# grantjr1842/delayed-streams-modeling

Measured on AMD Instinct MI355X. Metric: real-time stream throughput, stt-1b-en_fr @ bs=64 per GPU (Mimi encode + LM decode per 80 ms frame), higher is better.
Workload: dtype bf16 weights + bf16 KV, f32 activations as three exact bf16 pieces, f32 accumulate (v_mfma_f32_16x16x32_bf16); 1 GPU; stt-1b-en_fr batch=64 streaming, ring KV cache full (750 frames), Mimi encode + LM decode HIP path; streams_per_gpu=64, parallelism=replicas x1 (independent stream batches, no per-step collective), streams=encoder stream || 2 LM group stream(s)

## Files before the change

delayed-streams-modeling_amd/csrc/dsm_device.h:

```cpp
#pragma once
#include <hip/hip_runtime.h>

#include <atomic>
#include <cstdarg>
#include <cstdio>
#include <cstdlib>
#include <deque>
#include <mutex>
#include <shared_mutex>
#include <string>
#include <vector>

#include "../../include/dsm.h"
#include "dsm_gemm_plan.h"

#define HIPCHK_E(eng, expr)                                                                         \
  do {                                                                                              \
    hipError_t _e = (expr);                                                                         \
    if (_e != hipSuccess) {                                                                         \
      (eng)->set_error("%s failed: %s (%s:%d)", #expr, hipGetErrorString(_e), __FILE__, __LINE__);  \
      return DSM_ERR_DEVICE;                                                                        \
    }                                                                                               \
  } while (0)
#define HIPCHK(expr) HIPCHK_E(e, expr)

static void dsm_read_env(struct DsmDevice* e, bool stt);

struct DsmDevice {
  int device = 0;
  bool opened = false;
  hipStream_t s_enc = nullptr, s_model = nullptr;
  static constexpr int kMaxGroups = 4;
  hipStream_t s_grp[kMaxGroups] = {nullptr, nullptr, nullptr, nullptr};
  hipEvent_t ev_fork = nullptr, ev_grp_done[kMaxGroups] = {};
  bool prio_streams = false;
  int prio_hi = 0;
  bool use_graphs = true;
  bool fuse_qkv = true;
  bool stream_prio = false;
  bool fuse_front = true;
  int chunk_loop_min_tiles = GemmKnobs().chunk_loop_min_tiles;
  int loop_depth = GemmKnobs().loop_depth;
  int smallk_min_tiles = GemmKnobs().smallk_min_tiles;
  int smallk_mt = GemmKnobs().smallk_mt;
  size_t attn_lds_pad = 60000;
  int dot_mode = 0;

  int open(int device_id, int dot_mode_, bool stt) {
    device = device_id;
    dot_mode = dot_mode_;
    int ndev = 0;
    if (hipGetDeviceCount(&ndev) != hipSuccess || ndev <= device_id) {
      set_error("no usable HIP device %d (found %d): libdsm_mi355x has no CPU fallback", device_id, ndev);
      return DSM_ERR_DEVICE;
    }
    HIPCHK_E(this, hipSetDevice(device_id));
    opened = true;
    dsm_read_env(this, stt);
    prio_streams = stt;
    int prio_lo = 0;
    if (stt && stream_prio) (void)hipDeviceGetStreamPriorityRange(&prio_lo, &prio_hi);
    if (int rc = new_stream(&s_enc, prio_lo)) return rc;
    return new_stream(&s_model, prio_hi);
  }
  int new_stream(hipStream_t* out, int prio) {
    HIPCHK_E(this, prio_streams ? hipStreamCreateWithPriority(out, hipStreamNonBlocking, prio)
                                : hipStreamCreateWithFlags(out, hipStreamNonBlocking));
    return 0;
  }
  int open_groups(int G) {
    for (int g = 1; g < G; ++g) {
      if (int rc = new_stream(&s_grp[g], prio_hi)) return rc;
      if (int rc = new_event(&ev_grp_done[g])) return rc;
    }
    return new_event(&ev_fork);
  }
  int sid(hipStream_t st) const {
    if (st == s_enc) return 0;
    for (int g = 1; g < kMaxGroups; ++g)
      if (st == s_grp[g]) return 1 + g;
    return 1;
  }

  std::mutex own_mu;
  std::vector<void*> allocs, pinned;
  std::vector<hipEvent_t> events;
  template <typename T>
  int dalloc(T** out, size_t count, bool zero = true) {
    void* p = nullptr;
    size_t bytes = count * sizeof(T) + 256;
    HIPCHK_E(this, hipMalloc(&p, bytes));
    {
      std::lock_guard<std::mutex> lk(own_mu);
      allocs.push_back(p);
    }
    if (zero) {
      HIPCHK_E(this, hipMemset(p, 0, bytes));
      HIPCHK_E(this, hipStreamSynchronize(nullptr));
    }
    *out = reinterpret_cast<T*>(p);
    return 0;
  }
  template <typename T>
  int upload(T** out, const T* host, size_t count) {
    if (int rc = dalloc(out, count)) return rc;
    HIPCHK_E(this, hipMemcpy(*out, host, count * sizeof(T), hipMemcpyHostToDevice));
    HIPCHK_E(this, hipStreamSynchronize(nullptr));
    return 0;
  }
  template <typename T>
  int halloc(T** out, size_t count) {
    void* p = nullptr;
    HIPCHK_E(this, hipHostMalloc(&p, count * sizeof(T)));
    std::lock_guard<std::mutex> lk(own_mu);
    pinned.push_back(p);
    *out = reinterpret_cast<T*>(p);
    return 0;
  }
  int new_event(hipEvent_t* out, unsigned flags = hipEventDisableTiming) {
    HIPCHK_E(this, hipEventCreateWithFlags(out, flags));
    std::lock_guard<std::mutex> lk(own_mu);
    events.push_back(*out);
    return 0;
// ... 178 lines not shown
```

delayed-streams-modeling_amd/csrc/dsm_engine.hip:

```cpp
#include <hip/hip_runtime.h>

#include <cmath>
#include <cstdarg>
#include <cstdio>
#include <cstdlib>
#include <cstring>
#include <atomic>
#include <mutex>
#include <shared_mutex>
#include <string>
#include <set>
#include <vector>

#include "../../include/dsm.h"
#include "dsm_device.h"
#include "dsm_config_presets.h"
#include "dsm_gemm_plan.h"
#include "dsm_kernels.h"
#include "dsm_numerics.h"
#include "dsm_safetensors.h"

static thread_local std::string g_create_error;

static int dsm_env_int(const char* name, int dflt) {
  const char* v = getenv(name);
  return v ? atoi(v) : dflt;
}
static void dsm_read_env(DsmDevice* e, bool stt) {
  e->chunk_loop_min_tiles = gemm_default_knobs(stt, e->dot_mode).chunk_loop_min_tiles;
  if (stt && e->dot_mode == 1) e->attn_lds_pad = 40000;
  e->use_graphs = dsm_env_int("DSM_GRAPHS", 1) != 0;
  e->fuse_qkv = dsm_env_int("DSM_FUSE_QKV", 1) != 0;
  e->stream_prio = dsm_env_int("DSM_STREAM_PRIO", 0) != 0;
  e->fuse_front = dsm_env_int("DSM_FUSE_FRONT", 1) != 0;
  e->chunk_loop_min_tiles = dsm_env_int("DSM_CHUNK_LOOP_MIN", e->chunk_loop_min_tiles);
  e->loop_depth = dsm_env_int("DSM_LOOP_DEPTH", e->loop_depth) == 2 ? 2 : 4;
  e->smallk_min_tiles = dsm_env_int("DSM_SMALLK_MIN", e->smallk_min_tiles);
  const int mt = dsm_env_int("DSM_SMALLK_MT", e->smallk_mt);
  if (mt == 1 || mt == 2 || mt == 4) e->smallk_mt = mt;
}


namespace {

struct Linear {
  void* w = nullptr;
  float* bias = nullptr;
  int N = 0, K = 0, Npad = 0, Kpad = 0;
  bool bf16 = false;
  bool packed = false;
};

struct ConvGeom {
  Linear lin;
  int in_c = 0, out_c = 0, k = 0, stride = 1;
  int S = 0;
  int T_in = 0;
  int T_out = 0;
  bool replicate = false;
};

ConvGeom over_frames(const ConvGeom& g, int r) {
  ConvGeom c = g;
  c.T_in *= r;
  c.T_out *= r;
  return c;
}

struct TLayerW {
  Linear in_proj, out_proj, ff_in, ff_out;
  float *n1w = nullptr, *n1b = nullptr, *n2w = nullptr, *n2b = nullptr, *ls1 = nullptr, *ls2 = nullptr;
  Linear ca_q, ca_kv, ca_out;
  float *ncw = nullptr, *ncb = nullptr;
};

struct TransformerW {
  dsm_transformer_config cfg{};
  int hidden = 0;
  std::vector<TLayerW> layers;
  float* inv_freq = nullptr;
  bool rope_pos_before = false;
  bool has_ca = false;
  int ca_norm_rms = 0;
};

struct CaState {
  std::vector<void*> k, v;
  uint32_t* last = nullptr;
  uint8_t* act = nullptr;
  float* att = nullptr;
  int smax = 0;
};

struct TransformerState {
  std::vector<void*> k, v;
  uint32_t *pos = nullptr, *idx = nullptr, *start_pos = nullptr, *widx = nullptr;
  float* rope_cs = nullptr;
};

struct RvqW {
  Linear input_proj, output_proj;
  int n_q = 0;
  std::vector<Linear> codebooks;
};

struct MimiW {
  dsm_mimi_config cfg{};
  ConvGeom init_conv, final_conv, downsample;
  struct Stage {
    ConvGeom ra, rb, down;
  };
  std::vector<Stage> stages;
  TransformerW tr;
  RvqW rvq_first, rvq_rest;
  struct DecStage {
    Linear up;
    float* up_bias = nullptr;
    int in_c = 0, out_c = 0, k = 0, stride = 0, T_in = 0;
    ConvGeom ra, rb;
  };
  bool has_decoder = false;
  ConvGeom dec_init, dec_final;
  std::vector<DecStage> dec_stages;
  TransformerW dec_tr;
  float* upsample_w = nullptr;
  const float** emb_ptrs = nullptr;
};

struct ActScratch {
  float *x = nullptr, *xn = nullptr, *q = nullptr, *att = nullptr, *g = nullptr;
  ActScratch from_row(size_t r0, int d, int hid) const { return {x + r0 * d, xn + r0 * d, q + r0 * d, att + r0 * d, g + r0 * hid}; }
};

struct SeanetEnc {
  float* cat_init = nullptr;
  struct Stage {
    float *y = nullptr, *cat_ra = nullptr, *cat_rb = nullptr, *cat_down = nullptr;
  };
  std::vector<Stage> stages;
  float* cat_final = nullptr;
};

struct MimiState {
  float* pcm = nullptr;
  SeanetEnc enc;
  ActScratch act;
  float* cat_ds = nullptr;
  float* latent = nullptr;
  float *res_first = nullptr, *res_rest = nullptr, *pval = nullptr;
  uint32_t* pidx = nullptr;
  uint32_t* codes = nullptr;
  TransformerState tr;
  ConvStateDesc* descs = nullptr;
  std::vector<ConvStateDesc> h_descs;
  int ds_desc = -1;
  bool first_call = true;
  uint8_t* mask = nullptr;
};

struct MimiDecState {
  bool ready = false, first_call = true;
  DsmDevice::GraphSlot* graph = nullptr;
  float* h_pcm_out = nullptr;
  uint32_t* codes = nullptr;
  uint8_t* mask = nullptr;
  uint8_t* started = nullptr;
  float *q_first = nullptr, *q_rest = nullptr, *emb = nullptr, *up_carry = nullptr;
  ActScratch act;
  TransformerState tr;
  float* cat_init = nullptr;
  struct Stage {
    float *x = nullptr, *z = nullptr, *carry = nullptr, *y = nullptr, *cat_ra = nullptr, *cat_rb = nullptr;
  };
  std::vector<Stage> stages;
  float* cat_final = nullptr;
  float* pcm = nullptr;
  ConvStateDesc* descs = nullptr;
  std::vector<ConvStateDesc> h_descs;
};

struct LmW {
  uint16_t* text_emb = nullptr;
  uint16_t* audio_emb = nullptr;
  TransformerW tr;
  float* out_norm = nullptr;
  Linear text_linear, extra_heads;
};

struct LmState {
  ActScratch act;
  float *hidden = nullptr, *logits = nullptr, *eh = nullptr, *prs = nullptr;
  uint32_t *next_cb = nullptr, *text_token = nullptr, *text_out = nullptr, *codes_in = nullptr;
  uint8_t *first_step = nullptr, *mask = nullptr;
  uint32_t* rng_key = nullptr;
  unsigned long long* rng_pos = nullptr;
  uint8_t* gmask = nullptr;
  TransformerState tr;
  struct Group {
    int b0 = 0, nb = 0;
    TransformerState view;
  };
  std::vector<Group> groups;
};

struct HostItem {
  size_t step_idx = 0;
  std::vector<uint32_t> word_tokens;
  bool unended_word = false;
  double last_stop_time = 0.0;
};

}

struct dsm_engine : DsmDevice {
  dsm_asr_config cfg{};
  int B = 0;
  hipEvent_t ev_grp_in[kMaxGroups] = {}, ev_stagger[kMaxGroups] = {};
  bool grp_busy = false;
  bool serialize_groups = false;
  hipEvent_t ev_codes_consumed = nullptr;
  bool codes_consumed_valid = false;
  hipEvent_t ev_join = nullptr, ev_a = nullptr, ev_b = nullptr, ev_c = nullptr, ev_d = nullptr;
  MimiW mimi_w;
  MimiState mimi[2];
  std::atomic<bool> mimi1_ready{false};
  std::mutex mimi1_mu;
  MimiDecState dec;
  LmW lm_w;
  LmState lm;
  GraphSlot *g_enc[2] = {}, *g_grp[kMaxGroups] = {};
  float* h_pcm = nullptr;
// ... 787 lines not shown
```

delayed-streams-modeling_amd/csrc/dsm_engine_api.inc:

```

namespace {

template <typename KVT, int HD, int T>
int launch_attn_t(DsmDevice* e, hipStream_t st, float* out, const float* q, const void* k, const void* v,
                  const uint32_t* start_pos, const uint8_t* active, int B, int H, int ctx, int d, const AttnFused& fq) {
  constexpr int UNR = (sizeof(KVT) == 2 && T == 1 && HD == 128) ? 8 : 4;
  size_t lds = sizeof(float) * ((size_t)T * ctx + 4 * T * HD + 16);
  if ((long)B * H >= 2048 && (size_t)2 * ctx * HD * sizeof(KVT) >= (size_t)256 * 1024) lds += e->attn_lds_pad;
  if (lds > 64 * 1024) {
    static size_t allowed = 0;
    if (lds > allowed) {
      HIPCHK(hipFuncSetAttribute(reinterpret_cast<const void*>(&attn_kernel<KVT, HD, T, UNR>), hipFuncAttributeMaxDynamicSharedMemorySize, (int)lds));
      allowed = lds;
    }
  }
  const int tag = e->tag_attn[e->sid(st)];
  if (T == 1 && HD == 64 && ctx <= 32) {
    const int ph = e->prof_begin(tag, st);
    hipLaunchKernelGGL((attn_small_kernel<KVT, 64>), dim3((B * H + 3) / 4), dim3(256), 0, st, out, q, reinterpret_cast<const KVT*>(k),
                       reinterpret_cast<const KVT*>(v), start_pos, active, B * H, H, ctx, d, fq);
    e->prof_end(ph, st);
    HIPCHK(hipGetLastError());
    return 0;
  }
// ... 71 lines not shown
    a.act = 1;
    a.Y = act.g; a.ymap = plain_map(M, w.hidden);
    if (int rc = gemm_store<WT>(e, st, a)) return rc;
  }
  GemmArgs a = base_args(L.ff_out, act.g, plain_map(M, w.hidden), M);
  a.scale = L.ls2;
  a.res = act.x; a.rmap = plain_map(M, d);
  if (last && final_out) {
    a.Y = final_out; a.ymap = final_map;
  } else {
    a.Y = act.x; a.ymap = plain_map(M, d);
  }
  if (!last) set_norm(a, w.layers[l + 1].n1w, w.layers[l + 1].n1b, act.xn, c.norm);
  else if (post_norm_out) set_norm(a, post_norm_w, nullptr, post_norm_out, c.norm);
  return gemm_store<WT>(e, st, a);
}

template <typename WT, typename KVT>
int transformer_forward(DsmDevice* e, hipStream_t st, const TransformerW& w, TransformerState& s, const ActScratch& act, int B,
                        int T, const uint8_t* d_mask, float* final_out, RowMap final_map, const float* post_norm_w = nullptr,
                        float* post_norm_out = nullptr, int phase = 0, const CaState* ca = nullptr, bool head_done = false) {
  const dsm_transformer_config& c = w.cfg;
  const int d = c.d_model, H = c.num_heads, hd = d / H, M = B * T;
  if (phase != 2 && !head_done) {
    hipLaunchKernelGGL(kv_builder_kernel, dim3(B), dim3(64), 0, st, s.pos, s.idx, d_mask, s.start_pos, s.widx,
                       c.positional_embedding == 1 ? s.rope_cs : (float*)nullptr, w.inv_freq, B, T, c.context, hd,
                       w.rope_pos_before ? 1 : 0);
    HIPCHK(hipGetLastError());
    if (int rc = run_norm(e, st, act.xn, act.x, w.layers[0].n1w, w.layers[0].n1b, M, d, c.norm)) return rc;
  }
  for (int l = 0; l < c.num_layers; ++l) {
    const TLayerW& L = w.layers[l];
    AttnFused fq{};
    fq.nt = sizeof(KVT) == 2;
    if (!(phase == 2 && l == 0)) {
      GemmArgs a = base_args(L.in_proj, act.xn, plain_map(M, d), M);
      a.Y = act.q;
      a.d = d; a.hd = hd; a.H = H; a.T = T; a.ctx = c.context;
      a.kcache = s.k[l]; a.vcache = s.v[l];
      a.widx = s.widx;
      a.rope_cs = c.positional_embedding == 1 ? s.rope_cs : nullptr;
      a.active = d_mask;
      Slabs sl;
      if (int rc = launch_gemm<WT, KVT, EPI_QKV, 1>(e, st, a, true, T == 1 && e->fuse_qkv ? &sl : nullptr)) return rc;
      if (sl.ws) {
        fq.ws = sl.ws; fq.ld = sl.ld; fq.cstride = sl.cstride; fq.chunks = sl.chunks;
        fq.rope_cs = a.rope_cs;
        fq.widx = s.widx;
      }
      if (int rc = launch_attn<KVT>(e, st, act.att, act.q, s.k[l], s.v[l], s.start_pos, d_mask, B, H, hd, T, c.context, d, fq)) return rc;
    }
    if (phase == 1) return 0;
    if (int rc = transformer_layer_tail<WT, KVT>(e, st, w, l, act, B, T, final_out, final_map, post_norm_w, post_norm_out, ca)) return rc;
  }
  return 0;
}

template <typename F>
int with_kv_type(bool kv_bf16, F&& f) {
  return kv_bf16 ? f(uint16_t{}) : f(float{});
}

int fork_groups(DsmDevice* e, hipStream_t st, size_t G) {
  if (G > 1) {
    HIPCHK(hipEventRecord(e->ev_fork, st));
    for (size_t g = 1; g < G; ++g) HIPCHK(hipStreamWaitEvent(e->s_grp[g], e->ev_fork, 0));
  }
  return 0;
}
template <typename F>
int run_groups(DsmDevice* e, hipStream_t st, size_t G, bool serialize, F&& body) {
  for (size_t g = G; g-- > 0;) {
    hipStream_t gs = (g == 0 || serialize) ? st : e->s_grp[g];
    if (int rc = body(g, gs)) return rc;
    if (g > 0) HIPCHK(hipEventRecord(e->ev_grp_done[g], gs));
  }
  return 0;
}
int join_groups(DsmDevice* e, hipStream_t st, size_t G) {
  for (size_t g = 1; g < G; ++g) HIPCHK(hipStreamWaitEvent(st, e->ev_grp_done[g], 0));
  return 0;
}

int seanet_encode(DsmDevice* e, hipStream_t st, const MimiW& w, SeanetEnc& s, const float* cat_init, int B, int r, float* out,
                  RowMap omap, bool front_done = false) {
  const RowMap none = plain_map(1, 1);
  const size_t n = w.stages.size();
  const ConvGeom g0 = over_frames(w.init_conv, r), gf = over_frames(w.final_conv, r);
  if (!front_done)
    if (int rc = run_conv(e, st, g0, cat_init, B, s.stages[0].y, plain_map(B * g0.T_out, g0.out_c), s.stages[0].cat_ra,
                          cat_map(over_frames(w.stages[0].ra, r)), nullptr, none))
      return rc;
  for (size_t i = 0; i < n; ++i) {
    const ConvGeom ra = over_frames(w.stages[i].ra, r), rb = over_frames(w.stages[i].rb, r), dn = over_frames(w.stages[i].down, r);
    SeanetEnc::Stage& ss = s.stages[i];
    if (!(i == 0 && front_done)) {
      if (int rc = run_conv(e, st, ra, ss.cat_ra, B, nullptr, none, ss.cat_rb, cat_map(rb), nullptr, none)) return rc;
      if (int rc = run_conv(e, st, rb, ss.cat_rb, B, nullptr, none, ss.cat_down, cat_map(dn), ss.y, plain_map(B * rb.T_out, rb.out_c)))
        return rc;
    }
    if (i + 1 < n) {
      if (int rc = run_conv(e, st, dn, ss.cat_down, B, s.stages[i + 1].y, plain_map(B * dn.T_out, dn.out_c), s.stages[i + 1].cat_ra,
                            cat_map(over_frames(w.stages[i + 1].ra, r)), nullptr, none))
        return rc;
    } else if (int rc = run_conv(e, st, dn, ss.cat_down, B, nullptr, none, s.cat_final, cat_map(gf), nullptr, none)) {
      return rc;
    }
  }
  return run_conv(e, st, gf, s.cat_final, B, out, omap, nullptr, none, nullptr, none);
}

int mimi_encode_body(dsm_engine* e, int side, hipStream_t st);
int mimi_encode(dsm_engine* e, int side, hipStream_t st) {
  return run_captured(e, *e->g_enc[side], st, (uint64_t)e->sid(st), [&] { return mimi_encode_body(e, side, st); });
}
int mimi_encode_body(dsm_engine* e, int side, hipStream_t st) {
  const MimiW& w = e->mimi_w;
  MimiState& s = e->mimi[side];
  const int B = e->B;
  const RowMap none = plain_map(1, 1);
  e->tag_gemm[e->sid(st)] = DSM_PROF_GEMM_MIMI;
  e->tag_attn[e->sid(st)] = DSM_PROF_ATTN_MIMI;
  bool fused_front = false;
  {
    const MimiW::Stage& s0 = w.stages[0];
    const ConvGeom& c = w.init_conv;
    fused_front = e->fuse_front && c.in_c == 1 && c.k == 7 && c.stride == 1 && c.out_c == 64 && c.S == 6 && !c.lin.bf16 &&
                  s0.ra.k == 3 && s0.ra.stride == 1 && s0.ra.in_c == 64 && s0.ra.out_c == 32 && s0.ra.S == 2 && !s0.ra.lin.bf16 &&
                  s0.rb.k == 1 && s0.rb.stride == 1 && s0.rb.in_c == 32 && s0.rb.out_c == 64 && !s0.rb.lin.bf16 &&
                  c.T_in % 64 == 0 && c.T_out == c.T_in && s0.ra.T_in == c.T_in && s0.rb.T_in == c.T_in && s0.down.in_c == 64 &&
                  s0.down.T_in == c.T_in && !c.replicate && !s0.ra.replicate;
    if (fused_front) {
      SeanetFrontArgs fa;
      fa.cat_init = s.enc.cat_init;
      fa.w0 = reinterpret_cast<const float*>(c.lin.w); fa.b0 = c.lin.bias; fa.ld0 = c.lin.Kpad;
      fa.w1 = reinterpret_cast<const float*>(s0.ra.lin.w); fa.b1 = s0.ra.lin.bias; fa.ld1 = s0.ra.lin.Kpad;
      fa.w2 = reinterpret_cast<const float*>(s0.rb.lin.w); fa.b2 = s0.rb.lin.bias; fa.ld2 = s0.rb.lin.Kpad;
      fa.cat_ra = s.enc.stages[0].cat_ra;
      fa.cat_down = s.enc.stages[0].cat_down;
      fa.T = c.T_in; fa.S0 = c.S; fa.Sd = s0.down.S;
      const int ph = e->prof_begin(e->tag_gemm[e->sid(st)], st);
      hipLaunchKernelGGL(seanet_front_kernel<64>, dim3(c.T_in / 64, B), dim3(256), seanet_front_lds<64>(), st, fa);
      e->prof_end(ph, st);
      HIPCHK(hipGetLastError());
    }
  }
  const int Tt = w.final_conv.T_out, d = w.cfg.dimension;
  if (int rc = seanet_encode(e, st, w, s.enc, s.enc.cat_init, B, 1, s.act.x, plain_map(B * Tt, d), fused_front)) return rc;
  if (int rc = transformer_forward<float, float>(e, st, w.tr, s.tr, s.act, B, Tt, s.mask, s.cat_ds, cat_map(w.downsample))) return rc;
  if (s.first_call && w.downsample.S > 0) {
    hipLaunchKernelGGL(conv_replicate_init_kernel, dim3(B), dim3(256), 0, st, s.h_descs[s.ds_desc]);
    HIPCHK(hipGetLastError());
  }
  if (int rc = run_conv(e, st, w.downsample, s.cat_ds, B, s.latent, plain_map(B, d), nullptr, none, nullptr, none)) return rc;
  const int n_q = w.cfg.quantizer_n_q, qd = w.cfg.quantizer_dim;
  e->tag_gemm[e->sid(st)] = DSM_PROF_RVQ;
  for (int which = 0; which < 2; ++which) {
    const RvqW& r = which == 0 ? w.rvq_first : w.rvq_rest;
    if (r.n_q == 0) continue;
    float* res = which == 0 ? s.res_first : s.res_rest;
    {
      GemmArgs a = base_args(r.input_proj, s.latent, plain_map(B, d), B);
      a.Y = res; a.ymap = plain_map(B, qd);
      if (int rc = gemm_store<float>(e, st, a)) return rc;
    }
    for (int i = 0; i < r.n_q; ++i) {
      const Linear& cb = r.codebooks[i];
      GemmArgs a = base_args(cb, res, plain_map(B, qd), B);
      a.pval = s.pval; a.pidx = s.pidx;
      if (int rc = launch_gemm<float, float, EPI_RVQ, 1>(e, st, a, true)) return rc;
      hipLaunchKernelGGL(rvq_select_kernel, dim3(B), dim3(256), 0, st, s.pval, s.pidx, (cb.N + 15) / 16, B, s.codes, n_q,
                         which == 0 ? 0 : 1 + i, res, reinterpret_cast<const float*>(cb.w), qd, cb.Kpad);
      HIPCHK(hipGetLastError());
    }
  }
  if (!s.h_descs.empty()) {
    hipLaunchKernelGGL(conv_state_shift_kernel, dim3(B, (unsigned)s.h_descs.size()), dim3(256), 0, st, s.descs, s.mask,
                       s.first_call ? 1 : 0, nullptr);
    HIPCHK(hipGetLastError());
  }
  s.first_call = false;
  return 0;
}

int alloc_dec_state(DsmDevice* e, const MimiW& w, MimiDecState& s, int B) {
  if (s.ready) return 0;
  const dsm_mimi_config& c = w.cfg;
  const int dim = c.dimension, T2 = w.dec_init.T_in;
  if (!w.has_decoder) {
    e->set_error("the Mimi checkpoint has no decoder.* tensors: decode_step is unavailable");
    return DSM_ERR_STATE;
  }
  if (int rc = e->dalloc(&s.codes, (size_t)B * c.quantizer_n_q)) return rc;
  if (int rc = e->dalloc(&s.mask, B)) return rc;
  if (int rc = e->dalloc(&s.q_first, (size_t)B * c.quantizer_dim)) return rc;
  if (int rc = e->dalloc(&s.q_rest, (size_t)B * c.quantizer_dim)) return rc;
  if (int rc = e->dalloc(&s.emb, (size_t)B * dim)) return rc;
  if (int rc = e->dalloc(&s.up_carry, (size_t)B * c.downsample_stride * dim)) return rc;
  if (int rc = alloc_act(e, &s.act, (size_t)B * T2, dim, c.transformer.dim_feedforward)) return rc;
  if (int rc = alloc_transformer_state(e, &s.tr, c.transformer, B, T2, false)) return rc;
  auto add = [&](float* cat, const ConvGeom& g) { add_desc(s.h_descs, cat, g); };
  if (int rc = alloc_cat(e, &s.cat_init, w.dec_init, B)) return rc;
  add(s.cat_init, w.dec_init);
  s.stages.resize(w.dec_stages.size());
  for (size_t i = 0; i < w.dec_stages.size(); ++i) {
    const MimiW::DecStage& st = w.dec_stages[i];
    MimiDecState::Stage& ss = s.stages[i];
    const int T_out = st.T_in * st.stride;
    if (int rc = e->dalloc(&ss.x, (size_t)B * st.T_in * st.in_c)) return rc;
    if (int rc = e->dalloc(&ss.z, (size_t)B * st.T_in * st.k * st.out_c)) return rc;
    if (int rc = e->dalloc(&ss.carry, (size_t)B * (st.k - st.stride) * st.out_c)) return rc;
    if (int rc = e->dalloc(&ss.y, (size_t)B * T_out * st.out_c)) return rc;
    if (int rc = alloc_cat(e, &ss.cat_ra, st.ra, B)) return rc;
    if (int rc = alloc_cat(e, &ss.cat_rb, st.rb, B)) return rc;
    add(ss.cat_ra, st.ra);
    add(ss.cat_rb, st.rb);
  }
  if (int rc = alloc_cat(e, &s.cat_final, w.dec_final, B)) return rc;
  add(s.cat_final, w.dec_final);
  if (int rc = e->dalloc(&s.pcm, (size_t)B * DSM_FRAME_SIZE * c.channels)) return rc;
  if (int rc = e->upload(&s.descs, s.h_descs.data(), s.h_descs.size())) return rc;
  if (int rc = e->halloc(&s.h_pcm_out, (size_t)B * DSM_FRAME_SIZE)) return rc;
  s.graph = e->graph_slot();
  s.ready = true;
  return 0;
}

int mimi_decode_body(DsmDevice* e, const MimiW& w, MimiDecState& s, int B, hipStream_t st);
int mimi_decode(DsmDevice* e, const MimiW& w, MimiDecState& s, int B, hipStream_t st) {
  return run_captured(e, *s.graph, st, (uint64_t)e->sid(st), [&] { return mimi_decode_body(e, w, s, B, st); });
}
// ... 1017 lines not shown
  return 0;
}

int dsm_prof_timeline(dsm_engine* e, int on) {
  if (!e) return DSM_ERR_INVALID;
  e->timeline = on != 0;
  return 0;
}

int dsm_prof_timeline_read(dsm_engine* e, int* sid, int* kind, int* tag, double* start_us, double* end_us, int cap) {
  if (!e) return DSM_ERR_INVALID;
  HIPCHK(hipSetDevice(e->device));
  ApiShared api(e);
  if (int rc = dsm_sync(e)) return rc;
  const size_t n = e->dev_ts_tags.size();
  int out = 0;
  if (n) {
    std::vector<unsigned long long> h(2 * n);
    HIPCHK(hipMemcpy(h.data(), e->dev_ts, sizeof(unsigned long long) * 2 * n, hipMemcpyDeviceToHost));
    int khz = 100000;
    (void)hipDeviceGetAttribute(&khz, hipDeviceAttributeWallClockRate, e->device);
    unsigned long long t0 = ~0ull;
    for (size_t i = 0; i < n; ++i)
      if (h[2 * i + 1] >= h[2 * i] && h[2 * i] < t0) t0 = h[2 * i];
    for (size_t i = 0; i < n && out < cap; ++i) {
      if (h[2 * i + 1] < h[2 * i]) continue;
      sid[out] = e->dev_ts_info[i] >> 8;
      kind[out] = e->dev_ts_info[i] & 0xff;
      tag[out] = e->dev_ts_tags[i];
      start_us[out] = (double)(h[2 * i] - t0) * 1000.0 / khz;
      end_us[out] = (double)(h[2 * i + 1] - t0) * 1000.0 / khz;
      ++out;
    }
    for (size_t i = 0; i < n; ++i) { h[2 * i] = ~0ull; h[2 * i + 1] = 0; }
    HIPCHK(hipMemcpy(e->dev_ts, h.data(), sizeof(unsigned long long) * 2 * n, hipMemcpyHostToDevice));
    HIPCHK(hipStreamSynchronize(nullptr));
  }
  e->dev_ts_tags.clear();
  e->dev_ts_info.clear();
  return out;
}

int dsm_debug_set_positions(dsm_engine* e, uint32_t lm_pos, uint32_t mimi_pos) {
  if (!e) return DSM_ERR_INVALID;
  HIPCHK(hipSetDevice(e->device));
  ApiShared api(e);
  if (int rc = dsm_sync(e)) return rc;
  auto fill = [&](TransformerState& s, uint32_t pos, int ctx) {
    unsigned g = (unsigned)((e->B + 255) / 256);
    hipLaunchKernelGGL(fill_u32_kernel, dim3(g), dim3(256), 0, e->s_model, s.pos, pos, (long)e->B);
    hipLaunchKernelGGL(fill_u32_kernel, dim3(g), dim3(256), 0, e->s_model, s.idx, pos % (uint32_t)ctx, (long)e->B);
  };
  fill(e->lm.tr, lm_pos, e->cfg.lm.context);
  for (int side = 0; side < 2; ++side)
    if (side == 0 || e->mimi1_ready.load(std::memory_order_acquire)) fill(e->mimi[side].tr, mimi_pos, e->cfg.mimi.transformer.context);
  HIPCHK(hipGetLastError());
  return dsm_sync(e);
}

int dsm_debug_set_text_tokens(dsm_engine* e, const uint32_t* tokens) {
  if (!e || !tokens) return DSM_ERR_INVALID;
  HIPCHK(hipSetDevice(e->device));
  ApiShared api(e);
  if (int rc = dsm_sync(e)) return rc;
  HIPCHK(hipMemcpy(e->lm.text_token, tokens, sizeof(uint32_t) * (size_t)e->B, hipMemcpyHostToDevice));
  return dsm_sync(e);
}

int dsm_debug_read(dsm_engine* e, const char* name, float* out, size_t cap) {
  if (!e || !name || !out) return DSM_ERR_INVALID;
  HIPCHK(hipSetDevice(e->device));
  ApiShared api(e);
  if (int rc = dsm_sync(e)) return rc;
  const float* src = nullptr;
  size_t n = 0;
  const int B = e->B, dim = e->cfg.mimi.dimension;
  int side = 0;
  std::string nm(name);
  if (nm.rfind("mimi1.", 0) == 0) { side = 1; nm = nm.substr(6); }
  else if (nm.rfind("mimi.", 0) == 0) nm = nm.substr(5);
  if (nm == "lm.hidden") { src = e->lm.hidden; n = (size_t)B * e->cfg.lm.d_model; }
  else if (nm == "lm.logits") { src = e->lm.logits; n = (size_t)B * e->cfg.text_out_vocab_size; }
  else if (nm == "latent") { src = e->mimi[side].latent; n = (size_t)B * dim; }
  if (!src) { e->set_error("unknown debug tap %s", name); return DSM_ERR_INVALID; }
  if (n > cap) n = cap;
  HIPCHK(hipMemcpy(out, src, sizeof(float) * n, hipMemcpyDeviceToHost));
  return (int)n;
}

int dsm_debug_gemm_plan(int stt, int dot_mode, int weight_bf16, int epi, int nt, int M, int N, int K, int flags, char* buf, size_t cap) {
  if (epi < EPI_STORE || epi > EPI_RVQ || (nt != 1 && nt != 2) || M < 1 || N < 1 || K < 1 || !buf || !cap) return DSM_ERR_INVALID;
  GemmQuery q;
  q.weight_bf16 = weight_bf16 != 0;
  q.epi = epi;
  q.NT = nt;
  q.M = M; q.N = N; q.K = K;
  q.Kpad = round_up(K, 32);
  q.nt_stride = epi == EPI_GATE ? N : 16;
  q.aligned = flags & DSM_GEMMQ_ALIGNED;
  q.has_Y = flags & DSM_GEMMQ_Y; q.has_Y2 = flags & DSM_GEMMQ_Y2; q.has_res = flags & DSM_GEMMQ_RES;
  q.has_bias = flags & DSM_GEMMQ_BIAS; q.has_norm = flags & DSM_GEMMQ_NORM;
  q.y_ok4 = flags & DSM_GEMMQ_Y_OK4; q.y2_ok4 = flags & DSM_GEMMQ_Y2_OK4; q.res_ok4 = flags & DSM_GEMMQ_RES_OK4;
  q.y_bstride0 = flags & DSM_GEMMQ_Y_PLAIN;
  q.may_defer = flags & DSM_GEMMQ_MAY_DEFER;
  return gemm_plan_line(plan_gemm(q, gemm_default_knobs(stt != 0, dot_mode)), q.has_norm, buf, cap);
}

}
```

delayed-streams-modeling_amd/csrc/dsm_kernels.h:

```cpp
#pragma once
#include <hip/hip_runtime.h>
#include <stdint.h>
#include "dsm_numerics.h"
#include "dsm_sampling.h"

typedef float f32x4 __attribute__((ext_vector_type(4)));
typedef short dsm_bf16x8 __attribute__((ext_vector_type(8)));

__device__ __forceinline__ float wave_sum64(float v) {
#pragma unroll
  for (int off = 32; off >= 1; off >>= 1) v = v + __shfl_xor(v, off, 64);
  return v;
}

enum { EPI_STORE = 0, EPI_QKV = 1, EPI_GATE = 2, EPI_RVQ = 3 };

struct RowMap {
  long bstride;
  int rpb;
  int ld;
  int toff;
  __host__ __device__ long off(int m) const { return (long)(m / rpb) * bstride + (long)((m % rpb) + toff) * ld; }
};

// ... 1774 lines not shown
      float xr[TAPS0];
#pragma unroll
      for (int sidx = 0; sidx < TAPS0; ++sidx) xr[sidx] = xs[R + sidx];
      float yv[4];
#pragma unroll
      for (int j = 0; j < 4; ++j) {
        float acc = 0.0f;
#pragma unroll
        for (int sidx = 0; sidx < TAPS0; ++sidx) acc = dsm_unpaired(DSM_FMAF(w0r[j][sidx], xr[sidx], acc));
        yv[j] = a.b0 ? dsm_unpaired(acc + b0r[j]) : acc;
      }
      ev = make_float4(dsm_elu(yv[0]), dsm_elu(yv[1]), dsm_elu(yv[2]), dsm_elu(yv[3]));
      if (R >= 2) *reinterpret_cast<float4*>(&y0[(R - 2) * C0 + 4 * (cq ^ ((R - 2) & 15))]) = make_float4(yv[0], yv[1], yv[2], yv[3]);
      if (last && R >= TM)
        *reinterpret_cast<float4*>(a.cat_ra + ((long)b * (2 + a.T) + 2 + (t0 - 2 + R)) * C0 + 4 * cq) = ev;
    }
    *reinterpret_cast<float4*>(&e0[R * C0 + 4 * (cq ^ (R & 15))]) = ev;
  }
  __syncthreads();
  {
    constexpr int MPW = MTILES / 2;
    const int nt = wave & 1, mh = wave >> 1;
    f32x4 acc[MPW];
#pragma unroll
    for (int m2 = 0; m2 < MPW; ++m2) acc[m2] = (f32x4){0.f, 0.f, 0.f, 0.f};
    const float* wrow = a.w1 + (long)(16 * nt + r) * a.ld1 + 8 * q;
#pragma unroll
    for (int blk = 0; blk < 6; ++blk) {
      float wa[8], xb[MPW][8];
      load_w8<float>(wrow + 32 * blk, wa);
      const int tap = blk >> 1, u0 = (blk & 1) * 8 + 2 * q;
#pragma unroll
      for (int m2 = 0; m2 < MPW; ++m2) {
        const int R = 16 * (MPW * mh + m2) + r + tap;
        const float4 f0 = *reinterpret_cast<const float4*>(&e0[R * C0 + 4 * (u0 ^ (R & 15))]);
        const float4 f1 = *reinterpret_cast<const float4*>(&e0[R * C0 + 4 * ((u0 + 1) ^ (R & 15))]);
        xb[m2][0] = f0.x; xb[m2][1] = f0.y; xb[m2][2] = f0.z; xb[m2][3] = f0.w;
        xb[m2][4] = f1.x; xb[m2][5] = f1.y; xb[m2][6] = f1.z; xb[m2][7] = f1.w;
      }
#pragma unroll
      for (int sidx = 0; sidx < 8; ++sidx)
#pragma unroll
        for (int m2 = 0; m2 < MPW; ++m2) acc[m2] = __builtin_amdgcn_mfma_f32_16x16x4f32(wa[sidx], xb[m2][sidx], acc[m2], 0, 0, 0);
    }
#pragma unroll
    for (int m2 = 0; m2 < MPW; ++m2) {
      const int m = 16 * (MPW * mh + m2) + r, n = 16 * nt + 4 * q;
      float o[4];
#pragma unroll
      for (int i = 0; i < 4; ++i) o[i] = dsm_elu(a.b1 ? acc[m2][i] + a.b1[n + i] : acc[m2][i]);
      *reinterpret_cast<float4*>(&hs[m * C1 + 4 * ((n >> 2) ^ dsm_xs_sw(m))]) = make_float4(o[0], o[1], o[2], o[3]);
    }
  }
  __syncthreads();
  {
    f32x4 acc[MTILES];
#pragma unroll
    for (int mt = 0; mt < MTILES; ++mt) acc[mt] = (f32x4){0.f, 0.f, 0.f, 0.f};
    float wa[8], xb[MTILES][8];
    load_w8<float>(a.w2 + (long)(16 * wave + r) * a.ld2 + 8 * q, wa);
    const int xu0 = 4 * ((2 * q) ^ dsm_xs_sw(r)), xu1 = xu0 ^ 4;
#pragma unroll
    for (int mt = 0; mt < MTILES; ++mt) {
      const float* fp = &hs[(16 * mt + r) * C1];
      const float4 f0 = *reinterpret_cast<const float4*>(fp + xu0), f1 = *reinterpret_cast<const float4*>(fp + xu1);
      xb[mt][0] = f0.x; xb[mt][1] = f0.y; xb[mt][2] = f0.z; xb[mt][3] = f0.w;
      xb[mt][4] = f1.x; xb[mt][5] = f1.y; xb[mt][6] = f1.z; xb[mt][7] = f1.w;
    }
#pragma unroll
    for (int sidx = 0; sidx < 8; ++sidx)
#pragma unroll
      for (int mt = 0; mt < MTILES; ++mt) acc[mt] = __builtin_amdgcn_mfma_f32_16x16x4f32(wa[sidx], xb[mt][sidx], acc[mt], 0, 0, 0);
    float* out = a.cat_down + ((long)b * (a.Sd + a.T) + a.Sd + t0) * C0;
#pragma unroll
    for (int mt = 0; mt < MTILES; ++mt) {
      const int m = 16 * mt + r, n = 16 * wave + 4 * q;
      const float4 rv = *reinterpret_cast<const float4*>(&y0[m * C0 + 4 * ((n >> 2) ^ (m & 15))]);
      float o[4];
#pragma unroll
      for (int i = 0; i < 4; ++i) o[i] = a.b2 ? acc[mt][i] + a.b2[n + i] : acc[mt][i];
      o[0] = rv.x + o[0]; o[1] = rv.y + o[1]; o[2] = rv.z + o[2]; o[3] = rv.w + o[3];
      *reinterpret_cast<float4*>(out + (long)m * C0 + n) = make_float4(dsm_elu(o[0]), dsm_elu(o[1]), dsm_elu(o[2]), dsm_elu(o[3]));
    }
  }
}

struct ConvStateDesc {
  float* cat;
  long bstride;
  int S, T, C, replicate;
};

__global__ void conv_state_shift_kernel(const ConvStateDesc* __restrict__ descs, const uint8_t* __restrict__ active,
                                        int first_call, uint8_t* __restrict__ started) {
  const ConvStateDesc dsc = descs[blockIdx.y];
  const int b = blockIdx.x;
  float* base = dsc.cat + (long)b * dsc.bstride;
  const int n = dsc.S * dsc.C;
  if (active[b]) {
    const float* src = base + (long)dsc.T * dsc.C;
    for (int i = threadIdx.x; i < n; i += blockDim.x) base[i] = src[i];
    if (started && blockIdx.y == 0 && threadIdx.x == 0) started[b] = 1;
  } else if (first_call && !started) {
    for (int i = threadIdx.x; i < n; i += blockDim.x) base[i] = 0.0f;
  }
}

__global__ void conv_replicate_init_kernel(ConvStateDesc dsc) {
  const int b = blockIdx.x;
  float* base = dsc.cat + (long)b * dsc.bstride;
  const float* first = base + (long)dsc.S * dsc.C;
  for (int i = threadIdx.x; i < dsc.S * dsc.C; i += blockDim.x) base[i] = first[i % dsc.C];
}

__global__ void conv_state_reset_kernel(const ConvStateDesc* __restrict__ descs, int slot) {
  const ConvStateDesc dsc = descs[blockIdx.x];
  float* base = dsc.cat + (long)slot * dsc.bstride;
  for (int i = threadIdx.x; i < dsc.S * dsc.C; i += blockDim.x) base[i] = 0.0f;
}

__global__ void rvq_select_kernel(const float* __restrict__ pval, const uint32_t* __restrict__ pidx, int n_tiles,
                                  int M, uint32_t* __restrict__ codes, int code_stride, int code_off,
                                  float* __restrict__ residual, const float* __restrict__ E, int dim, int ldE) {
  const int m = blockIdx.x;
  __shared__ uint32_t s_code;
  if (threadIdx.x < 64) {
    float bv = DSM_INF_F;
    uint32_t bi = 0xFFFFFFFFu;
    for (int t = threadIdx.x; t < n_tiles; t += 64) {
      float v = pval[(long)t * M + m];
      uint32_t i = pidx[(long)t * M + m];
      if (v < bv || (v == bv && i < bi)) { bv = v; bi = i; }
    }
#pragma unroll
    for (int off = 32; off >= 1; off >>= 1) {
      float ov = __shfl_xor(bv, off, 64);
      uint32_t oi = __shfl_xor(bi, off, 64);
      if (ov < bv || (ov == bv && oi < bi)) { bv = ov; bi = oi; }
    }
    if (threadIdx.x == 0) {
      s_code = bi;
      codes[(long)m * code_stride + code_off] = bi;
    }
  }
  __syncthreads();
  const uint32_t c = s_code;
  for (int i = threadIdx.x; i < dim; i += blockDim.x)
    residual[(long)m * dim + i] = residual[(long)m * dim + i] - E[(long)c * ldE + i];
}

struct RvqGatherArgs {
  const float* const* emb;
  int n_q, bins, dim, ldE;
};
__global__ void rvq_gather_sum_kernel(RvqGatherArgs a, const uint32_t* __restrict__ codes, float* __restrict__ q_first,
                                      float* __restrict__ q_rest) {
  const int b = blockIdx.x;
  for (int dd = threadIdx.x; dd < a.dim; dd += blockDim.x) {
    uint32_t c0 = codes[b * a.n_q];
    c0 = c0 < (uint32_t)a.bins ? c0 : 0u;
    q_first[(long)b * a.dim + dd] = a.emb[0][(long)c0 * a.ldE + dd];
    float acc = 0.0f;
    for (int i = 1; i < a.n_q; ++i) {
      uint32_t c = codes[b * a.n_q + i];
      c = c < (uint32_t)a.bins ? c : 0u;
      float ev = a.emb[i][(long)c * a.ldE + dd];
// ... 269 lines not shown
```

Baseline: 1869 x realtime (stream-seconds of audio per wall second).

## Fuse SEANet residual block convs into one LDS-resident kernel for later stages

Adds a seanet_resblock_kernel that runs the k=3 conv, ELU, k=1 conv, bias, skip add and ELU of a SEANet residual block in one launch. The intermediate hidden activations stay in LDS instead of passing through global memory, and the two run_conv launches per stage become one. It is used for stages after the first when channels are 128 or 256 with fp32 weights, and is on by default via DSM_FUSE_STAGES. It also adds a seanet_out debug tap that copies the encoder output only when requested, and the fused kernel's summation order may differ slightly from the unfused path.

```diff
diff --git a/delayed-streams-modeling_amd/csrc/dsm_device.h b/delayed-streams-modeling_amd/csrc/dsm_device.h
--- a/delayed-streams-modeling_amd/csrc/dsm_device.h
+++ b/delayed-streams-modeling_amd/csrc/dsm_device.h
@@ -39,6 +39,7 @@
   bool fuse_qkv = true;
   bool stream_prio = false;
   bool fuse_front = true;
+  bool fuse_stages = true;
   int chunk_loop_min_tiles = GemmKnobs().chunk_loop_min_tiles;
   int loop_depth = GemmKnobs().loop_depth;
   int smallk_min_tiles = GemmKnobs().smallk_min_tiles;
diff --git a/delayed-streams-modeling_amd/csrc/dsm_engine.hip b/delayed-streams-modeling_amd/csrc/dsm_engine.hip
--- a/delayed-streams-modeling_amd/csrc/dsm_engine.hip
+++ b/delayed-streams-modeling_amd/csrc/dsm_engine.hip
@@ -33,6 +33,7 @@
   e->fuse_qkv = dsm_env_int("DSM_FUSE_QKV", 1) != 0;
   e->stream_prio = dsm_env_int("DSM_STREAM_PRIO", 0) != 0;
   e->fuse_front = dsm_env_int("DSM_FUSE_FRONT", 1) != 0;
+  e->fuse_stages = dsm_env_int("DSM_FUSE_STAGES", 1) != 0;
   e->chunk_loop_min_tiles = dsm_env_int("DSM_CHUNK_LOOP_MIN", e->chunk_loop_min_tiles);
   e->loop_depth = dsm_env_int("DSM_LOOP_DEPTH", e->loop_depth) == 2 ? 2 : 4;
   e->smallk_min_tiles = dsm_env_int("DSM_SMALLK_MIN", e->smallk_min_tiles);
@@ -147,6 +148,7 @@
   ActScratch act;
   float* cat_ds = nullptr;
   float* latent = nullptr;
+  float* dbg_seanet = nullptr;
   float *res_first = nullptr, *res_rest = nullptr, *pval = nullptr;
   uint32_t* pidx = nullptr;
   uint32_t* codes = nullptr;
diff --git a/delayed-streams-modeling_amd/csrc/dsm_engine_api.inc b/delayed-streams-modeling_amd/csrc/dsm_engine_api.inc
--- a/delayed-streams-modeling_amd/csrc/dsm_engine_api.inc
+++ b/delayed-streams-modeling_amd/csrc/dsm_engine_api.inc
@@ -177,8 +177,34 @@
   return 0;
 }
 
+template <int C, int TM>
+int launch_resblock_form(DsmDevice* e, hipStream_t st, const SeanetResblockArgs& ra, int B) {
+  const int ph = e->prof_begin(e->tag_gemm[e->sid(st)], st);
+  const size_t lds = seanet_resblock_lds<C, TM>();
+  hipLaunchKernelGGL((seanet_resblock_kernel<C, TM>), dim3(ra.T / TM, B), dim3(256), lds, st, ra);
+  e->prof_end(ph, st);
+  HIPCHK(hipGetLastError());
+  return 0;
+}
+int launch_resblock(DsmDevice* e, hipStream_t st, const ConvGeom& ra, const ConvGeom& rb, const ConvGeom& dn,
+                    const SeanetEnc::Stage& ss, int B, bool* done) {
+  const int C = ra.in_c, TM = 32;
+  *done = (C == 128 || C == 256) && !ra.lin.bf16 && !rb.lin.bf16 &&
+          ra.k == 3 && ra.stride == 1 && ra.S == 2 && ra.out_c == C / 2 && !ra.replicate && ra.T_out == ra.T_in &&
+          rb.k == 1 && rb.stride == 1 && rb.S == 0 && rb.in_c == C / 2 && rb.out_c == C && rb.T_in == ra.T_in && rb.T_out == ra.T_in &&
+          dn.in_c == C && dn.T_in == ra.T_in && ra.T_in % TM == 0 && ra.lin.Kpad >= 3 * C && rb.lin.Kpad >= C / 2;
+  if (!*done) return 0;
+  SeanetResblockArgs a;
+  a.cat_ra = ss.cat_ra;
+  a.skip = ss.y;
+  a.wa = reinterpret_cast<const float*>(ra.lin.w); a.ba = ra.lin.bias; a.lda = ra.lin.Kpad;
+  a.wb = reinterpret_cast<const float*>(rb.lin.w); a.bb = rb.lin.bias; a.ldb = rb.lin.Kpad;
+  a.cat_down = ss.cat_down;
+  a.T = ra.T_in; a.Sd = dn.S;
+  return C == 128 ? launch_resblock_form<128, 32>(e, st, a, B) : launch_resblock_form<256, 32>(e, st, a, B);
+}
 int seanet_encode(DsmDevice* e, hipStream_t st, const MimiW& w, SeanetEnc& s, const float* cat_init, int B, int r, float* out,
-                  RowMap omap, bool front_done = false) {
+                  RowMap omap, bool front_done = false, bool fuse_stages = false) {
   const RowMap none = plain_map(1, 1);
   const size_t n = w.stages.size();
   const ConvGeom g0 = over_frames(w.init_conv, r), gf = over_frames(w.final_conv, r);
@@ -189,7 +215,10 @@
   for (size_t i = 0; i < n; ++i) {
     const ConvGeom ra = over_frames(w.stages[i].ra, r), rb = over_frames(w.stages[i].rb, r), dn = over_frames(w.stages[i].down, r);
     SeanetEnc::Stage& ss = s.stages[i];
-    if (!(i == 0 && front_done)) {
+    bool block_done = i == 0 && front_done;
+    if (!block_done && fuse_stages && i > 0)
+      if (int rc = launch_resblock(e, st, ra, rb, dn, ss, B, &block_done)) return rc;
+    if (!block_done) {
       if (int rc = run_conv(e, st, ra, ss.cat_ra, B, nullptr, none, ss.cat_rb, cat_map(rb), nullptr, none)) return rc;
       if (int rc = run_conv(e, st, rb, ss.cat_rb, B, nullptr, none, ss.cat_down, cat_map(dn), ss.y, plain_map(B * rb.T_out, rb.out_c)))
         return rc;
@@ -241,7 +270,9 @@
     }
   }
   const int Tt = w.final_conv.T_out, d = w.cfg.dimension;
-  if (int rc = seanet_encode(e, st, w, s.enc, s.enc.cat_init, B, 1, s.act.x, plain_map(B * Tt, d), fused_front)) return rc;
+  if (int rc = seanet_encode(e, st, w, s.enc, s.enc.cat_init, B, 1, s.act.x, plain_map(B * Tt, d), fused_front, e->fuse_stages)) return rc;
+  if (s.dbg_seanet)
+    HIPCHK(hipMemcpyAsync(s.dbg_seanet, s.act.x, sizeof(float) * (size_t)B * Tt * d, hipMemcpyDeviceToDevice, st));
   if (int rc = transformer_forward<float, float>(e, st, w.tr, s.tr, s.act, B, Tt, s.mask, s.cat_ds, cat_map(w.downsample))) return rc;
   if (s.first_call && w.downsample.S > 0) {
     hipLaunchKernelGGL(conv_replicate_init_kernel, dim3(B), dim3(256), 0, st, s.h_descs[s.ds_desc]);
@@ -1425,6 +1456,15 @@
   if (nm == "lm.hidden") { src = e->lm.hidden; n = (size_t)B * e->cfg.lm.d_model; }
   else if (nm == "lm.logits") { src = e->lm.logits; n = (size_t)B * e->cfg.text_out_vocab_size; }
   else if (nm == "latent") { src = e->mimi[side].latent; n = (size_t)B * dim; }
+  else if (nm == "seanet_out") {
+    MimiState& ms = e->mimi[side];
+    n = (size_t)B * e->mimi_w.final_conv.T_out * dim;
+    if (!ms.dbg_seanet) {
+      if (int rc = e->dalloc(&ms.dbg_seanet, n)) return rc;
+      e->ws_gen += 1;
+    }
+    src = ms.dbg_seanet;
+  }
   if (!src) { e->set_error("unknown debug tap %s", name); return DSM_ERR_INVALID; }
   if (n > cap) n = cap;
   HIPCHK(hipMemcpy(out, src, sizeof(float) * n, hipMemcpyDeviceToHost));
diff --git a/delayed-streams-modeling_amd/csrc/dsm_kernels.h b/delayed-streams-modeling_amd/csrc/dsm_kernels.h
--- a/delayed-streams-modeling_amd/csrc/dsm_kernels.h
+++ b/delayed-streams-modeling_amd/csrc/dsm_kernels.h
@@ -1880,6 +1880,181 @@
       o[0] = rv.x + o[0]; o[1] = rv.y + o[1]; o[2] = rv.z + o[2]; o[3] = rv.w + o[3];
       *reinterpret_cast<float4*>(out + (long)m * C0 + n) = make_float4(dsm_elu(o[0]), dsm_elu(o[1]), dsm_elu(o[2]), dsm_elu(o[3]));
     }
+  }
+}
+
+struct SeanetResblockArgs {
+  const float* cat_ra;
+  const float* skip;
+  const float *wa, *ba;
+  const float *wb, *bb;
+  float* cat_down;
+  int lda, ldb;
+  int T, Sd;
+};
+
+__device__ __forceinline__ void resblock_frag(const float* row, int R, int u0, float (&o)[8]) {
+  const float4 f0 = *reinterpret_cast<const float4*>(row + 4 * (u0 ^ (R & 15)));
+  const float4 f1 = *reinterpret_cast<const float4*>(row + 4 * ((u0 + 1) ^ (R & 15)));
+  o[0] = f0.x; o[1] = f0.y; o[2] = f0.z; o[3] = f0.w; o[4] = f1.x; o[5] = f1.y; o[6] = f1.z; o[7] = f1.w;
+}
+
+template <int C, int TM>
+constexpr size_t seanet_resblock_lds() { return sizeof(float) * ((TM + 2) * C + TM * (C / 2)); }
+template <int C, int TM>
+__global__ __launch_bounds__(256) void seanet_resblock_kernel(SeanetResblockArgs a) {
+  static_assert((C == 128 || C == 256) && TM % 16 == 0 && TM <= 64, "geometry");
+  constexpr int CH = C / 2, MT = TM / 16, UR = C / 4;
+  constexpr int NTA = CH / 64, NBA = 3 * C / 32;
+  constexpr int NTB = C / 64, NBB = CH / 32;
+  constexpr int D = NTA == 1 ? 4 : 2;
+  extern __shared__ __attribute__((aligned(16))) float resblock_lds[];
+  float* es = resblock_lds;
+  float* hs = es + (TM + 2) * C;
+  const int tid = threadIdx.x, lane = tid & 63, wave = tid >> 6;
+  const int r = lane & 15, q = lane >> 4;
+  const int b = blockIdx.y, t0 = blockIdx.x * TM;
+  const float* wrow[NTA];
+  Raw8<float> rw[D][NTA];
+#pragma unroll
+  for (int j = 0; j < NTA; ++j) wrow[j] = a.wa + (long)(16 * (wave + 4 * j) + r) * a.lda + 8 * q;
+#pragma unroll
+  for (int d = 0; d < D; ++d)
+#pragma unroll
+    for (int j = 0; j < NTA; ++j) rw[d][j].load(wrow[j] + 32 * d);
+  {
+    const float* src = a.cat_ra + ((long)b * (2 + a.T) + t0) * C;
+    constexpr int NU = (TM + 2) * UR, NL = (NU + 255) / 256;
+    float4 v[NL];
+#pragma unroll
+    for (int k = 0; k < NL; ++k) v[k] = *reinterpret_cast<const float4*>(src + 4 * (long)min(tid + 256 * k, NU - 1));
+#pragma unroll
+    for (int k = 0; k < NL; ++k) {
+      const int i = tid + 256 * k, R = i / UR, u = i % UR;
+      if (i < NU) *reinterpret_cast<float4*>(&es[R * C + 4 * (u ^ (R & 15))]) = v[k];
+    }
+  }
+  __syncthreads();
+  {
+    f32x4 acc[NTA][MT], tot[NTA][MT];
+#pragma unroll
+    for (int j = 0; j < NTA; ++j)
+#pragma unroll
+      for (int mt = 0; mt < MT; ++mt) {
+        acc[j][mt] = (f32x4){0.f, 0.f, 0.f, 0.f};
+        tot[j][mt] = (f32x4){0.f, 0.f, 0.f, 0.f};
+      }
+    float xb[2][MT][8], ba4[NTA][4];
+#pragma unroll
+    for (int j = 0; j < NTA; ++j)
+#pragma unroll
+      for (int i = 0; i < 4; ++i) ba4[j][i] = a.ba ? a.ba[16 * (wave + 4 * j) + 4 * q + i] : 0.0f;
+#pragma unroll
+    for (int mt = 0; mt < MT; ++mt) resblock_frag(es + (16 * mt + r) * C, 16 * mt + r, 2 * q, xb[0][mt]);
+#pragma unroll
+    for (int blk = 0; blk < NBA; ++blk) {
+      float w8[NTA][8];
+      __builtin_amdgcn_sched_barrier(0);
+#pragma unroll
+      for (int j = 0; j < NTA; ++j) {
+        rw[blk % D][j].unpack(w8[j]);
+        if (blk + D < NBA) rw[blk % D][j].load(wrow[j] + 32 * (blk + D));
+      }
+      __builtin_amdgcn_sched_barrier(0);
+#pragma unroll
+      for (int s = 0; s < 8; ++s) {
+#pragma unroll
+        for (int j = 0; j < NTA; ++j)
+#pragma unroll
+          for (int mt = 0; mt < MT; ++mt)
+            acc[j][mt] = __builtin_amdgcn_mfma_f32_16x16x4f32(w8[j][s], xb[blk & 1][mt][s], acc[j][mt], 0, 0, 0);
+        if (s == 0) {
+          if (blk + 1 < NBA) {
+            const int tap = (32 * (blk + 1)) / C, u0 = ((32 * (blk + 1)) % C) / 4 + 2 * q;
+#pragma unroll
+            for (int mt = 0; mt < MT; ++mt) resblock_frag(es + (16 * mt + r + tap) * C, 16 * mt + r + tap, u0, xb[(blk + 1) & 1][mt]);
+          }
+          __builtin_amdgcn_sched_barrier(0);
+        }
+      }
+      if ((blk & 7) == 7 || blk == NBA - 1) {
+#pragma unroll
+        for (int j = 0; j < NTA; ++j)
+#pragma unroll
+          for (int mt = 0; mt < MT; ++mt)
+#pragma unroll
+            for (int i = 0; i < 4; ++i) {
+              tot[j][mt][i] = dsm_unpaired(tot[j][mt][i] + acc[j][mt][i]);
+              acc[j][mt][i] = 0.f;
+            }
+      }
+    }
+#pragma unroll
+    for (int j = 0; j < NTA; ++j)
+#pragma unroll
+      for (int mt = 0; mt < MT; ++mt) {
+        const int m = 16 * mt + r, n = 16 * (wave + 4 * j) + 4 * q;
+        float o[4];
+#pragma unroll
+        for (int i = 0; i < 4; ++i) o[i] = dsm_elu(a.ba ? dsm_unpaired(tot[j][mt][i] + ba4[j][i]) : tot[j][mt][i]);
+        *reinterpret_cast<float4*>(&hs[m * CH + 4 * ((n >> 2) ^ (m & 15))]) = make_float4(o[0], o[1], o[2], o[3]);
+      }
+  }
+  {
+    const float* skip = a.skip + ((long)b * a.T + t0) * C;
+    float* out = a.cat_down + ((long)b * (a.Sd + a.T) + a.Sd + t0) * C;
+    Raw8<float> rb[NBB];
+    float4 rv[MT];
+    float bv[4];
+#define DSM_RB_LOAD(J)                                                                                     \
+  {                                                                                                         \
+    const float* wr_ = a.wb + (long)(16 * (wave + 4 * (J)) + r) * a.ldb + 8 * q;                            \
+    _Pragma("unroll") for (int blk = 0; blk < NBB; ++blk) rb[blk].load(wr_ + 32 * blk);                     \
+    _Pragma("unroll") for (int mt = 0; mt < MT; ++mt)                                                       \
+      rv[mt] = *reinterpret_cast<const float4*>(skip + (long)(16 * mt + r) * C + 16 * (wave + 4 * (J)) + 4 * q); \
+    _Pragma("unroll") for (int i = 0; i < 4; ++i) bv[i] = a.bb ? a.bb[16 * (wave + 4 * (J)) + 4 * q + i] : 0.0f; \
+  }
+    DSM_RB_LOAD(0)
+    __syncthreads();
+    float xb[NBB][MT][8];
+#pragma unroll
+    for (int blk = 0; blk < NBB; ++blk)
+#pragma unroll
+      for (int mt = 0; mt < MT; ++mt) resblock_frag(hs + (16 * mt + r) * CH, 16 * mt + r, 8 * blk + 2 * q, xb[blk][mt]);
+#pragma unroll
+    for (int j = 0; j < NTB; ++j) {
+      const int n = 16 * (wave + 4 * j) + 4 * q;
+      float w8[NBB][8], rs[MT][4], bs[4];
+      __builtin_amdgcn_sched_barrier(0);
+#pragma unroll
+      for (int blk = 0; blk < NBB; ++blk) rb[blk].unpack(w8[blk]);
+#pragma unroll
+      for (int mt = 0; mt < MT; ++mt) { rs[mt][0] = rv[mt].x; rs[mt][1] = rv[mt].y; rs[mt][2] = rv[mt].z; rs[mt][3] = rv[mt].w; }
+#pragma unroll
+      for (int i = 0; i < 4; ++i) bs[i] = bv[i];
+      if (j + 1 < NTB) DSM_RB_LOAD(j + 1)
+      __builtin_amdgcn_sched_barrier(0);
+      f32x4 acc[MT];
+#pragma unroll
+      for (int mt = 0; mt < MT; ++mt) acc[mt] = (f32x4){0.f, 0.f, 0.f, 0.f};
+#pragma unroll
+      for (int blk = 0; blk < NBB; ++blk)
+#pragma unroll
+        for (int s = 0; s < 8; ++s)
+#pragma unroll
+          for (int mt = 0; mt < MT; ++mt) acc[mt] = __builtin_amdgcn_mfma_f32_16x16x4f32(w8[blk][s], xb[blk][mt][s], acc[mt], 0, 0, 0);
+#pragma unroll
+      for (int mt = 0; mt < MT; ++mt) {
+        float o[4];
+#pragma unroll
+        for (int i = 0; i < 4; ++i) {
+          const float t = a.bb ? dsm_unpaired(acc[mt][i] + bs[i]) : acc[mt][i];
+          o[i] = dsm_elu(dsm_unpaired(rs[mt][i] + t));
+        }
+        *reinterpret_cast<float4*>(out + (long)(16 * mt + r) * C + n) = make_float4(o[0], o[1], o[2], o[3]);
+      }
+    }
+#undef DSM_RB_LOAD
   }
 }
 
```

After: 1884 x realtime (stream-seconds of audio per wall second), median of 6. No clear change (+0.8%).
